# clementabary/music2dance

Measured on AMD Instinct MI355X. Metric: 120-frame seq/sec, phase3 WGAN-GP step, batch 64 per GPU, higher is better.
Workload: dtype f32

## Files before the change

music2dance_amd/build.py:

```python
import os
import shutil
import subprocess
import sys
from concurrent.futures import ThreadPoolExecutor

PKG_DIR = os.path.dirname(os.path.abspath(__file__))
CSRC = os.path.join(PKG_DIR, "csrc")
LIB_DIR = os.path.join(PKG_DIR, "lib")
LIB_PATH = os.path.join(LIB_DIR, "libm2d_hip.so")
SOURCES = ["m2d_runtime.hip", "gemm_engine.hip", "conv1d.hip", "tcn.hip", "probe_gemm.hip", "conv1d_thin.hip", "bn.hip", "gru.hip",
           "pointwise.hip", "cond.hip", "render.hip", "resample.hip", "spectral.hip"]
STAMPED = ["gemm_engine.hip", "tcn.hip"]
STAMP_LIB_PATH = os.path.join(LIB_DIR, "libm2d_hip_stamp.so")
FLAGS = ["--offload-arch=gfx950", "-O3", "-std=c++17", "-fPIC", "-ffp-contract=off", "-Wall",
         "-Wno-unused-function"] + os.environ.get("M2D_EXTRA_FLAGS", "").split()


def _hipcc():
    exe = shutil.which("hipcc") or "/opt/rocm/bin/hipcc"
    if not os.path.exists(exe):
        raise RuntimeError("hipcc not found: cannot build libm2d_hip.so")
    return exe


def _stale(target, deps):
    if not os.path.exists(target):
        return True
    t = os.path.getmtime(target)
    return any(os.path.getmtime(d) > t for d in deps)


def build(force=False, verbose=True, stamp=True):
    os.makedirs(LIB_DIR, exist_ok=True)
    obj_dir = os.path.join(LIB_DIR, "obj")
    os.makedirs(obj_dir, exist_ok=True)
    hipcc = _hipcc()
    headers = [os.path.join(CSRC, f) for f in os.listdir(CSRC) if f.endswith(".h")]
    jobs = []
    objs = []
    for src in SOURCES:
        s = os.path.join(CSRC, src)
        o = os.path.join(obj_dir, src.replace(".hip", ".o"))
        objs.append(o)
        if force or _stale(o, [s] + headers):
            jobs.append([hipcc] + FLAGS + ["-c", s, "-o", o])

    def run(cmd):
        if verbose:
            print("[m2d build]", " ".join(cmd), flush=True)
        r = subprocess.run(cmd, capture_output=True, text=True)
        if r.returncode != 0:
            raise RuntimeError("hipcc failed:\n%s\n%s" % (" ".join(cmd), r.stderr))
        return r

    sobjs = []
    sjobs = []
    if stamp:
        for src in SOURCES:
            if src in STAMPED:
                s = os.path.join(CSRC, src)
                o = os.path.join(obj_dir, src.replace(".hip", ".stamp.o"))
                sobjs.append(o)
                if force or _stale(o, [s] + headers):
                    sjobs.append([hipcc] + FLAGS + ["-DM2D_STAMP", "-c", s, "-o", o])
            else:
                sobjs.append(os.path.join(obj_dir, src.replace(".hip", ".o")))
    with ThreadPoolExecutor(max_workers=4) as ex:
        list(ex.map(run, jobs + sjobs))
    if force or jobs or _stale(LIB_PATH, objs):
        run([hipcc, "--offload-arch=gfx950", "-shared", "-fPIC", "-o", LIB_PATH] + objs)
    if stamp and (force or jobs or sjobs or _stale(STAMP_LIB_PATH, sobjs)):
        run([hipcc, "--offload-arch=gfx950", "-shared", "-fPIC", "-o", STAMP_LIB_PATH] + sobjs)
    return LIB_PATH


if __name__ == "__main__":
    build(force="--force" in sys.argv, stamp="--no-stamp" not in sys.argv)
    print(LIB_PATH)
```

music2dance_amd/csrc/conv1d.hip:

```cpp
#include "gemm_engine.h"
#include "tcn.h"

static inline int conv_out_len(int L, int ks, int stride, int pad) {
  const int span = L + 2 * pad - ks;
  return span < 0 ? 0 : span / stride + 1;
}

static inline bool fits_i32(long long v) { return v >= 0 && v < 2147483647LL; }

struct M2dWinView {
  int T, S, hop;
};
bool m2d_thin_applicable(int Cin, int Cout, int ks, int stride);
bool m2d_thin_long_applicable(int Cin, int Cout, int ks, int stride, int pad, int L);
size_t m2d_thin_long_stats_ws(int B, int Lout);
int m2d_thin_long_fwd(const float* x, const float* w, const float* bias, float* y, int B, int L, int ks, int stride, int pad,
                      int Lout, int act, float slope, const M2dWinView* wv, double* stats, void* ws, size_t ws_bytes,
                      hipStream_t stream);
size_t m2d_thin_bwd_weight_ws(int B, int Cout, int ks, int Lout);
size_t m2d_thin_fwd_stats_ws(int B, int Lout);
int m2d_thin_fwd(const float* x, const float* w, const float* bias, float* y, int B, int L, int Cout, int ks,
                 int stride, int pad, int Lout, int act, float slope, const float* out_mask, float out_mask_slope,
                 const M2dWinView* wv, double* stats, void* ws, size_t ws_bytes, hipStream_t stream);
int m2d_thin_bwd_data(const float* dy, const float* w, float* dx, int B, int L, int Cout, int ks, int stride,
                      int pad, int Lout, const float* dy_mask, float dy_mask_slope, hipStream_t stream);
int m2d_thin_bwd_weight(const float* x, const float* dy, float* dw, float* dbias, int B, int L, int Cout, int ks,
                        int stride, int pad, int Lout, const float* dy_mask, float dy_mask_slope, void* ws,
                        size_t ws_bytes, const M2dWinView* wv, hipStream_t stream);

static inline bool conv_uses_packed(int Cin) { return Cin >= M2D_BK; }
static inline float fwd_tile_penalty(int stride) { return stride > 1 ? 1.25f : 1.f; }

static void fill_fwd(M2dGemmParams& p, const float* x, const float* w, const float* wp, float* y, int B, int Cin,
                     int L, int Cout, int ks, int stride, int pad, int Lout, const M2dWinView* wv = nullptr) {
  memset(&p, 0, sizeof(p));
  p.M = Cout;
  p.N = B * Lout;
  p.K = Cin * ks;
  p.phases = 1;
  const bool packed = conv_uses_packed(Cin);
  M2dOperand& b = p.B;
  b.base = x;
  b.nbytes = m2d_extent_bytes((long long)B * Cin * L);
  b.nrows = p.N;
  b.rdiv = Lout;
  b.rdiv_inv = 1.f / (float)Lout;
  b.r_hi_stride = Cin * L;
  b.r_lo_stride = stride;
  b.r_off = -pad;
  b.r_pos_mul = stride;
  b.r_pos_off = -pad;
  b.lim = L;
  if (wv && wv->T > 0) {
    b.nbytes = m2d_extent_bytes((long long)(B / wv->T) * wv->S);
    b.r_hi_stride = wv->hop;
    b.rdiv2 = wv->T;
    b.rdiv2_inv = 1.f / (float)wv->T;
    b.r_hi2_stride = wv->S;
  }
  if (packed) {
    p.nhi = ks;
    p.kdiv = Cin;
    p.lo_outer = 1;
    p.small_tile_penalty = fwd_tile_penalty(stride);
    m2d_operand_plain(p.A, wp, Cout, 1, ks * Cout, (long long)Cout * Cin * ks);
    p.A.k_hi_stride = Cout;
    b.k_hi_stride = 1;
    b.k_lo_stride = L;
    b.k_pos_hi = 1;
    b.k_pos_lo = 0;
    b.k_safe_lo = 0;
    b.k_safe_hi = 0x7fffffff;
  } else {
    p.nhi = Cin;
    p.kdiv = ks;
    m2d_operand_plain(p.A, w, Cout, Cin * ks, 1, (long long)Cout * Cin * ks);
    p.A.k_hi_stride = ks;
    b.k_hi_stride = L;
    b.k_lo_stride = 1;
    b.k_pos_hi = 0;
    b.k_pos_lo = 1;
    b.k_safe_lo = pad;
    b.k_safe_hi = L - (Lout - 1) * stride + pad;
  }
  m2d_outmap_plain(p.O, y, Lout, 1);
  p.O.cdiv = Lout;
  p.O.cdiv_inv = 1.f / (float)Lout;
  p.O.c_hi_stride = Cout * Lout;
  p.O.c_lo_stride = 1;
}

__global__ void __launch_bounds__(256) m2d_pack_weights_kernel(const float* __restrict__ w, float* __restrict__ wf,
                                                                 float* __restrict__ wb, int Cout, int Cin, int ks) {
  const size_t total = (size_t)Cout * Cin * ks;
  for (size_t idx = (size_t)blockIdx.x * 256 + threadIdx.x; idx < total; idx += (size_t)gridDim.x * 256) {
    const int ci = (int)(idx % Cin);
    const size_t t = idx / Cin;
    const int kk = (int)(t % ks);
    const int co = (int)(t / ks);
    const float v = w[((size_t)co * Cin + ci) * ks + kk];
    if (wf) wf[idx] = v;
    if (wb) wb[((size_t)ci * ks + kk) * Cout + co] = v;
  }
}

__global__ void __launch_bounds__(256) m2d_pack_weights_subpixel_kernel(const float* __restrict__ w, float* __restrict__ out,
                                                                          int Cout, int Cin, int ks, int s, int nt, int phase_major) {
  const size_t total = (size_t)nt * Cout * Cin * s;
  for (size_t idx = (size_t)blockIdx.x * 256 + threadIdx.x; idx < total; idx += (size_t)gridDim.x * 256) {
    const int m = (int)(idx % (size_t)(Cin * s));
    const size_t k = idx / (size_t)(Cin * s);
    const int ci = phase_major ? (m / (32 * s)) * 32 + m % 32 : m / s, r = phase_major ? (m % (32 * s)) / 32 : m - ci * s;
    const int co = (int)(k % Cout), t = (int)(k / Cout);
    const int tap = r + s * t;
    out[idx] = tap < ks ? w[((size_t)co * Cin + ci) * ks + tap] : 0.f;
  }
}

static inline bool subpixel_tall(int Cin, int Cout, int ks, int stride);
static inline bool bwd_subpixel(int Cin, int Cout, int ks, int stride, bool masked_dy = false) {
  static const bool on = [] { const char* e = getenv("M2D_SUBPIXEL"); return !(e && e[0] == '0'); }();
  static const int max_rows = [] { const char* e = getenv("M2D_SUBPIXEL_MAXROWS"); return e ? atoi(e) : 128; }();
  static const int tall_max_cin = [] { const char* e = getenv("M2D_SUBPIXEL_TALL_MAXCIN"); return e ? atoi(e) : 64; }();
  if (on && !masked_dy && Cin > 32 && Cin <= tall_max_cin && subpixel_tall(Cin, Cout, ks, stride)) return true;
  return on && stride > 1 && Cin * stride <= max_rows && Cin * stride >= 64 && Cout >= 16 && ks > stride;
}
static inline bool subpixel_tall(int Cin, int Cout, int ks, int stride) {
  static const bool on = [] { const char* e = getenv("M2D_SUBPIXEL_TALL"); return !(e && e[0] == '0'); }();
  const int nt = (ks + stride - 1) / stride;
  return on && m2d_dl_enabled() && Cin % 32 == 0 && stride == 4 && ks - stride * (nt - 1) == 1 && nt >= 2;
}
static inline size_t subpixel_bytes(int Cout, int Cin, int ks, int stride) {
  return ((((size_t)((ks + stride - 1) / stride) * Cout * Cin * stride) * sizeof(float)) + 255) & ~(size_t)255;
}

static int pack_weights(const float* w, float* wf, float* wb, int Cout, int Cin, int ks, hipStream_t stream) {
  const size_t total = (size_t)Cout * Cin * ks;
  unsigned blocks = (unsigned)((total + 255) / 256);
  if (blocks > 4096) blocks = 4096;
  hipLaunchKernelGGL(m2d_pack_weights_kernel, dim3(blocks), dim3(256), 0, stream, w, wf, wb, Cout, Cin, ks);
  M2D_CHECK_LAUNCH("m2d_pack_weights_kernel");
  return M2D_OK;
}

static inline size_t pack_bytes(int Cout, int Cin, int ks) {
  return (((size_t)Cout * Cin * ks * sizeof(float)) + 255) & ~(size_t)255;
}

extern "C" {

int m2d_conv1d_pack_weights(const float* w, float* w_fwd, float* w_bwd, int Cout, int Cin, int ks, void* stream) {
  if (Cout <= 0 || Cin <= 0 || ks <= 0 || !w) M2D_FAIL(M2D_ERR_ARG, "m2d_conv1d_pack_weights: bad arguments");
  if (!fits_i32((long long)Cout * Cin * ks)) M2D_FAIL(M2D_ERR_RANGE, "m2d_conv1d_pack_weights: too large");
  if (!w_fwd && !w_bwd) return M2D_OK;
// ... 392 lines not shown
  if (stride == 1 && Lout == L && (mask_wrap % 4u) == 0) {
    const int nt = m2d_tcn_conv_tile(B, Cout, L, Cin, ks, stride, pad);
    if (nt > 0) {
      M2dTcnConv t;
      memset(&t, 0, sizeof(t));
      t.x = dy;
      t.x_mask = dy_mask;
      t.x_mask_slope = dy_mask_slope;
      t.wimg = w_packed;
      t.out = dx;
      t.out_mask = out_mask;
      t.out_mask_slope = out_mask_slope;
      t.out_mask_wrap = mask_wrap;
      t.residual = residual;
      t.mask_last = 1;
      t.tap_rev = 1;
      t.B = B;
      t.Cin = Cout;
      t.L = L;
      return m2d_tcn_conv_launch(t, ks, nt, (hipStream_t)stream, "m2d_conv1d_bwd_data");
    }
  }
  p.bwd_data = 1;
  p.plan_kind = stride > 1 ? M2D_PLAN_BWD_DATA : M2D_PLAN_GENERAL;
  p.phases = stride;
  p.ph_ks = ks;
  p.ph_cout = Cout;
  p.ph_pad = pad;
  p.ph_L = L;
  p.ph_batch = B;
  p.M = Cin;
  p.kdiv = Cout;
  p.lo_outer = 1;
  p.nhi = (ks + stride - 1) / stride;
  int nq_max = 0;
  for (int r = 0; r < stride; ++r) {
    const int qmin = r >= pad ? 0 : (pad - r + stride - 1) / stride;
    const int top = L - 1 + pad - r;
    const int nq = top >= 0 ? (top / stride - qmin + 1) : 0;
    if (nq > nq_max) nq_max = nq;
  }
  p.N = B * nq_max;
  p.K = Cout * p.nhi;
  m2d_operand_plain(p.A, w_packed, Cin, 1, ks * Cin, (long long)Cout * Cin * ks);
  p.A.k_hi_stride = stride * Cin;
  p.ph_a_step = Cin;
  M2dOperand& b = p.B;
  b.base = dy;
  b.nbytes = m2d_extent_bytes((long long)B * Cout * Lout);
  b.mask = dy_mask;
  b.mask_slope = dy_mask_slope;
  b.nrows = p.N;
  b.rdiv = nq_max;
  b.rdiv_inv = 1.f / (float)nq_max;
  b.r_hi_stride = Cout * Lout;
  b.r_lo_stride = 1;
  b.r_pos_mul = 1;
  b.k_hi_stride = -1;
  b.k_lo_stride = Lout;
  b.k_pos_hi = -1;
  b.k_pos_lo = 0;
  b.k_safe_lo = 0;
  b.k_safe_hi = 0x7fffffff;
  b.lim = Lout;
  m2d_outmap_plain(p.O, dx, L, 1);
  p.O.c_hi_stride = Cin * L;
  p.O.c_lo_stride = stride;
  p.O.c_pos_mul = stride;
  p.O.c_lim = L;
  p.O.mask = out_mask;
  p.O.mask_wrap = mask_wrap;
  p.O.mask_slope = out_mask_slope;
  p.O.residual = residual;
  p.O.mask_last = 1;
  if (stride == 1) {
    p.bwd_data = 0;
    p.phases = 1;
    p.N = B * L;
    p.nhi = ks;
    p.K = Cout * ks;
    b.nrows = p.N;
    b.rdiv = L;
    b.rdiv_inv = 1.f / (float)L;
    b.r_off = pad;
    b.r_pos_off = pad;
    p.O.cdiv = L;
    p.O.cdiv_inv = b.rdiv_inv;
    p.O.c_off = 0;
    p.O.c_pos_off = 0;
    p.O.c_lim = 0;
    return m2d_gemm_launch(p, false, false, true, ws, ws_bytes,
                           (hipStream_t)stream, "m2d_conv1d_bwd_data");
  }
  return m2d_gemm_launch(p, false, false, false, ws, ws_bytes,
                         (hipStream_t)stream, "m2d_conv1d_bwd_data");
}

int m2d_conv1d_bwd_data(const float* dy, const float* w, const float* w_packed, float* dx, int B, int Cin, int L,
                        int Cout, int ks, int stride, int pad, const float* dy_mask, float dy_mask_slope,
                        const float* out_mask, float out_mask_slope, void* ws, size_t ws_bytes, void* stream) {
  return conv1d_bwd_data_impl(dy, w, w_packed, dx, B, Cin, L, Cout, ks, stride, pad, dy_mask, dy_mask_slope, out_mask,
                              out_mask_slope, ws, ws_bytes, stream, nullptr);
}

int m2d_conv1d_bwd_data_res(const float* dy, const float* w, const float* w_packed, float* dx, int B, int Cin, int L,
                            int Cout, int ks, int stride, int pad, const float* dy_mask, float dy_mask_slope,
                            const float* residual, const float* out_mask, float out_mask_slope, void* ws,
                            size_t ws_bytes, void* stream) {
  return conv1d_bwd_data_impl(dy, w, w_packed, dx, B, Cin, L, Cout, ks, stride, pad, dy_mask, dy_mask_slope, out_mask,
                              out_mask_slope, ws, ws_bytes, stream, residual);
}

int m2d_conv1d_bwd_data_shared_mask(const float* dy, const float* w, const float* w_packed, float* dx, int B, int Cin,
                                    int L, int Cout, int ks, int stride, int pad, const float* out_mask,
                                    float out_mask_slope, int mask_batch, void* ws, size_t ws_bytes, void* stream) {
  if (m2d_thin_applicable(Cin, Cout, ks, stride))
    M2D_FAIL(M2D_ERR_ARG, "m2d_conv1d_bwd_data_shared_mask: not for the thin (Cin = 1) layer");
  return conv1d_bwd_data_impl(dy, w, w_packed, dx, B, Cin, L, Cout, ks, stride, pad, nullptr, 0.f, out_mask,
                              out_mask_slope, ws, ws_bytes, stream, nullptr, mask_batch);
}

static int conv1d_bwd_weight_impl(const float* x, const float* dy, float* dw, float* dbias, int B, int Cin, int L,
                                  int Cout, int ks, int stride, int pad, const float* dy_mask, float dy_mask_slope,
                                  void* ws, size_t ws_bytes, void* stream, const M2dWinView* wv,
                                  int bias_from_sample = 0) {
  const int Lout = conv_out_len(L, ks, stride, pad);
  if (bias_from_sample < 0 || bias_from_sample > B) M2D_FAIL(M2D_ERR_ARG, "m2d_conv1d_bwd_weight: bad bias_from_sample");
  if (bias_from_sample > 0 && dbias && (Lout < M2D_BK || m2d_thin_applicable(Cin, Cout, ks, stride)))
    M2D_FAIL(M2D_ERR_ARG, "m2d_conv1d_bwd_weight: bias_from_sample needs >= %d output positions and Cin > 1", M2D_BK);
  if (B <= 0 || Cin <= 0 || Cout <= 0 || Lout <= 0)
    M2D_FAIL(M2D_ERR_ARG, "m2d_conv1d_bwd_weight: bad shape");
  if (!fits_i32((long long)B * Cin * L) || !fits_i32((long long)B * Cout * Lout))
    M2D_FAIL(M2D_ERR_RANGE, "m2d_conv1d_bwd_weight: tensor exceeds 2^31 elements");
  if (m2d_thin_applicable(Cin, Cout, ks, stride))
    return m2d_thin_bwd_weight(x, dy, dw, dbias, B, L, Cout, ks, stride, pad, Lout, dy_mask, dy_mask_slope, ws,
                               ws_bytes, wv, (hipStream_t)stream);
  if (wv && (Cin != 1 || Lout < M2D_BK))
    M2D_FAIL(M2D_ERR_ARG, "m2d_conv1d_bwd_weight_windows: single-channel convs with >= %d output positions only", M2D_BK);
  if (!wv && Lout == L && m2d_tcn_wgrad_applicable(B, Cin, L, Cout, ks, stride, pad)) {
    M2dTcnWgrad t;
    memset(&t, 0, sizeof(t));
    t.x = x;
    t.dy = dy;
    t.dy_mask = dy_mask;
    t.dy_mask_slope = dy_mask_slope;
    t.dw = dw;
    t.dbias = dbias;
    t.bias_from = bias_from_sample;
    t.B = B;
    t.Cin = Cin;
    t.L = L;
    return m2d_tcn_wgrad_launch(t, ks, ws, ws_bytes, (hipStream_t)stream, "m2d_conv1d_bwd_weight");
  }
  M2dGemmParams p;
  memset(&p, 0, sizeof(p));
  p.M = Cout;
  p.N = Cin * ks;
  p.K = B * Lout;
  p.phases = 1;
  M2dOperand& b = p.B;
  b.base = x;
  b.nbytes = m2d_extent_bytes((long long)B * Cin * L);
  b.nrows = p.N;
  b.rdiv = ks;
  b.rdiv_inv = 1.f / (float)ks;
  b.r_hi_stride = L;
  b.r_lo_stride = 1;
  b.r_off = -pad;
  b.r_pos_mul = 1;
  b.r_pos_off = -pad;
  b.lim = L;
  bool a_kfast = true;
  if (Lout >= M2D_BK) {
    p.nhi = B;
    p.kdiv = Lout;
    m2d_operand_plain(p.A, dy, Cout, Lout, 1, (long long)B * Cout * Lout);
    p.A.k_hi_stride = Cout * Lout;
    b.k_hi_stride = Cin * L;
    b.k_lo_stride = stride;
    b.k_pos_hi = 0;
    b.k_pos_lo = stride;
    if (wv && wv->T > 0) {
      b.nbytes = m2d_extent_bytes((long long)(B / wv->T) * wv->S);
      b.k_hi_stride = wv->hop;
      b.kdiv2 = wv->T;
      b.k_hi2_stride = wv->S;
    }
    b.k_safe_lo = (pad + stride - 1) / stride;
    b.k_safe_hi = (L - ks + pad) >= 0 ? (L - ks + pad) / stride + 1 : 0;
    p.plan_kind = M2D_PLAN_BWD_WEIGHT;
  } else {
    p.nhi = Lout;
    p.kdiv = B;
    a_kfast = false;
    m2d_operand_plain(p.A, dy, Cout, Lout, Cout * Lout, (long long)B * Cout * Lout);
    p.A.k_hi_stride = 1;
    b.k_hi_stride = stride;
    b.k_lo_stride = Cin * L;
    b.k_pos_hi = stride;
    b.k_pos_lo = 0;
    b.k_safe_lo = 0;
    b.k_safe_hi = 0x7fffffff;
  }
  p.A.mask = dy_mask;
  p.A.mask_slope = dy_mask_slope;
  m2d_outmap_plain(p.O, dw, Cin * ks, 1);
  if (dbias) {
    p.N = Cin * ks + 1;
    b.ones_row_p1 = Cin * ks + 1;
    b.ones_from_hi = bias_from_sample;
    p.O.col_out = dbias;
    p.O.redirect_col_p1 = Cin * ks + 1;
  }
  return m2d_gemm_launch(p, a_kfast, false, true, ws, ws_bytes, (hipStream_t)stream,
                         "m2d_conv1d_bwd_weight");
}

int m2d_conv1d_bwd_weight(const float* x, const float* dy, float* dw, float* dbias, int B, int Cin, int L,
                          int Cout, int ks, int stride, int pad, const float* dy_mask, float dy_mask_slope,
                          void* ws, size_t ws_bytes, void* stream) {
  return conv1d_bwd_weight_impl(x, dy, dw, dbias, B, Cin, L, Cout, ks, stride, pad, dy_mask, dy_mask_slope, ws,
                                ws_bytes, stream, nullptr);
}

int m2d_conv1d_bwd_weight_from(const float* x, const float* dy, float* dw, float* dbias, int B, int Cin, int L,
                               int Cout, int ks, int stride, int pad, const float* dy_mask, float dy_mask_slope,
                               int bias_from_sample, void* ws, size_t ws_bytes, void* stream) {
  return conv1d_bwd_weight_impl(x, dy, dw, dbias, B, Cin, L, Cout, ks, stride, pad, dy_mask, dy_mask_slope, ws,
                                ws_bytes, stream, nullptr, bias_from_sample);
}

int m2d_conv1d_bwd_weight_windows(const float* track, int B, int S, int T, int hop, int window, const float* dy,
                                  float* dw, float* dbias, int Cout, int ks, int stride, int pad,
                                  const float* dy_mask, float dy_mask_slope, void* ws, size_t ws_bytes, void* stream) {
  if (B <= 0 || T <= 0 || hop <= 0 || window <= 0 || (long long)(T - 1) * hop + window > S)
    M2D_FAIL(M2D_ERR_ARG, "m2d_conv1d_bwd_weight_windows: windows do not fit the track");
  if (!fits_i32((long long)B * S) || !fits_i32((long long)B * T * window))
    M2D_FAIL(M2D_ERR_RANGE, "m2d_conv1d_bwd_weight_windows: tensor exceeds 2^31 elements");
  const M2dWinView wv = {T, S, hop};
  return conv1d_bwd_weight_impl(track, dy, dw, dbias, B * T, 1, window, Cout, ks, stride, pad, dy_mask, dy_mask_slope,
                                ws, ws_bytes, stream, &wv);
}

size_t m2d_conv1d_workspace_bytes(int which, int B, int Cin, int L, int Cout, int ks, int stride, int pad) {
  const int Lout = conv_out_len(L, ks, stride, pad);
  if (Lout <= 0) return 0;
  if (m2d_thin_applicable(Cin, Cout, ks, stride))
    return which == 2 ? m2d_thin_bwd_weight_ws(B, Cout, ks, Lout) : (which == 0 ? m2d_thin_fwd_stats_ws(B, Lout) : 0);
  if (which == 0 && m2d_thin_long_applicable(Cin, Cout, ks, stride, pad, L)) {
    const size_t a = m2d_gemm_plan(Cout, B * Lout, m2d_chunks(Cin, ks), 1, true).ws_bytes + m2d_rowstats_bytes(Cout, B * Lout);
    const size_t t = m2d_thin_long_stats_ws(B, Lout);
    return a > t ? a : t;
  }
  if (which == 0) {
    if (Lout == 1 && pad == 0 && L == ks) {
      const size_t a = m2d_gemm_plan(Cout, B, m2d_chunks(1, Cin * ks), 1, true).ws_bytes, st = m2d_rowstats_bytes(Cout, B);
      return a + st;
    }
    const bool packed = conv_uses_packed(Cin);
    const int nch = packed ? m2d_chunks(ks, Cin) : m2d_chunks(Cin, ks);
    const size_t a = m2d_gemm_plan(Cout, B * Lout, nch, 1, true, packed ? fwd_tile_penalty(stride) : 1.f).ws_bytes;
    const size_t st = m2d_rowstats_bytes(Cout, B * Lout);
    return a + st + (packed ? pack_bytes(Cout, Cin, ks) : 0);
  }
  if (which == 1) {
    if (Lout == 1 && pad == 0 && L == ks) return m2d_gemm_plan(B, Cin * ks, m2d_chunks(1, Cout), 1, true).ws_bytes;
    if (stride == 1) return m2d_gemm_plan(Cin, B * L, m2d_chunks(ks, Cout), 1, true).ws_bytes + pack_bytes(Cout, Cin, ks);
    if (bwd_subpixel(Cin, Cout, ks, stride)) return subpixel_bytes(Cout, Cin, ks, stride) + pack_bytes(Cout, Cin, ks);
    return pack_bytes(Cout, Cin, ks);
  }
  const int nch = Lout >= M2D_BK ? m2d_chunks(B, Lout) : m2d_chunks(Lout, B);
  const int kind = Lout >= M2D_BK ? M2D_PLAN_BWD_WEIGHT : M2D_PLAN_GENERAL;
  const size_t a = m2d_gemm_plan(Cout, Cin * ks, nch, 1, true, 1.0, kind).ws_bytes;
  const size_t c = m2d_gemm_plan(Cout, Cin * ks + 1, nch, 1, true, 1.0, kind).ws_bytes;
  const size_t t = (Lout == L && m2d_tcn_wgrad_applicable(B, Cin, L, Cout, ks, stride, pad)) ? m2d_tcn_wgrad_ws_bytes(B, Cin, L, ks) : 0;
  return (a > c ? a : c) > t ? (a > c ? a : c) : t;
}

static int gemm_impl(int mode, const float* a, int lda, const float* b, int ldb, const float* bias, float* c, int ldc,
                     int M, int N, int K, int act, float slope, const float* a_mask, float a_mask_slope,
                     const float* out_mask, float out_mask_slope, void* ws, size_t ws_bytes, void* stream) {
  if (M < 0 || N < 0 || K < 0 || mode < 0 || mode > 2) M2D_FAIL(M2D_ERR_ARG, "m2d_gemm: bad arguments");
  const int a_cols = mode == 2 ? M : K, b_cols = mode == 0 ? K : N;
  if (lda == 0) lda = a_cols;
  if (ldb == 0) ldb = b_cols;
  if (ldc == 0) ldc = N;
  if (lda < a_cols || ldb < b_cols || ldc < N) M2D_FAIL(M2D_ERR_ARG, "m2d_gemm: leading dimension smaller than the row");
  if (!fits_i32((long long)M * K) || !fits_i32((long long)N * K) || !fits_i32((long long)M * N))
    M2D_FAIL(M2D_ERR_RANGE, "m2d_gemm: matrix exceeds 2^31 elements");
  M2dGemmParams p;
  memset(&p, 0, sizeof(p));
  p.M = M;
  p.N = N;
  p.K = K;
  p.nhi = K > 0 ? 1 : 0;
  p.kdiv = K > 0 ? K : 1;
  p.phases = 1;
  bool akf = true, bkf = true;
  const long long a_rows = mode == 2 ? K : M, b_rows = mode == 0 ? N : K;
  const long long ea = K > 0 ? (a_rows - 1) * lda + a_cols : 1, eb = K > 0 ? (b_rows - 1) * ldb + b_cols : 1;
  if (!fits_i32((long long)(M - 1) * ldc + N)) M2D_FAIL(M2D_ERR_RANGE, "m2d_gemm: output exceeds 2^31 elements");
  if (mode == 0) {
    m2d_operand_plain(p.A, a, M, lda, 1, ea);
    m2d_operand_plain(p.B, b, N, ldb, 1, eb);
    akf = true;
    bkf = true;
  } else if (mode == 1) {
    m2d_operand_plain(p.A, a, M, lda, 1, ea);
    m2d_operand_plain(p.B, b, N, 1, ldb, eb);
    akf = true;
    bkf = false;
  } else {
    m2d_operand_plain(p.A, a, M, 1, lda, ea);
    m2d_operand_plain(p.B, b, N, 1, ldb, eb);
    akf = false;
    bkf = false;
  }
  p.A.mask = a_mask;
  p.A.mask_slope = a_mask_slope;
  m2d_outmap_plain(p.O, c, ldc, 1);
  p.O.bias = bias;
  p.O.bias_mode = bias ? 2 : 0;
  p.O.act = act;
  p.O.slope = slope;
  p.O.mask = out_mask;
  p.O.mask_slope = out_mask_slope;
  return m2d_gemm_launch(p, akf, bkf, true, ws, ws_bytes, (hipStream_t)stream, "m2d_gemm");
}

int m2d_gemm(int mode, const float* a, const float* b, const float* bias, float* c, int M, int N, int K,
             int act, float slope, const float* a_mask, float a_mask_slope, const float* out_mask,
             float out_mask_slope, void* ws, size_t ws_bytes, void* stream) {
  return gemm_impl(mode, a, 0, b, 0, bias, c, 0, M, N, K, act, slope, a_mask, a_mask_slope, out_mask, out_mask_slope,
                   ws, ws_bytes, stream);
}

int m2d_gemm_ld(int mode, const float* a, int lda, const float* b, int ldb, const float* bias, float* c, int ldc,
                int M, int N, int K, int act, float slope, const float* a_mask, float a_mask_slope,
                const float* out_mask, float out_mask_slope, void* ws, size_t ws_bytes, void* stream) {
  return gemm_impl(mode, a, lda, b, ldb, bias, c, ldc, M, N, K, act, slope, a_mask, a_mask_slope, out_mask,
                   out_mask_slope, ws, ws_bytes, stream);
}

size_t m2d_gemm_workspace_bytes(int mode, int M, int N, int K) {
  (void)mode;
  return m2d_gemm_plan(M, N, m2d_chunks(K > 0 ? 1 : 0, K > 0 ? K : 1), 1, true).ws_bytes;
}

}
```

Baseline: 5702.

## Add specialized MFMA weight-gradient kernel for k25 stride-4 conv1d

Adds a dedicated weight-gradient kernel for conv1d layers with kernel size 25, stride 4 and padding 11 (the WaveGAN-style discriminator shape). It uses fp32 32x32x2 MFMA with double-buffered LDS staging of dy and x chunks, buffer loads with out-of-bounds handling, and a per-run partial slab. A separate reduce kernel then sums the partials into dw and dbias. It replaces the generic GEMM-engine path for these shapes, adds workspace sizing for the new slab, and can be disabled with an env var. The cost is more code and a two-kernel split-K reduction.

After: 5731 (median of 6 runs). Within noise of the previous version (+0.5%).

```diff
diff --git a/music2dance_amd/build.py b/music2dance_amd/build.py
--- a/music2dance_amd/build.py
+++ b/music2dance_amd/build.py
@@ -8,7 +8,8 @@
 CSRC = os.path.join(PKG_DIR, "csrc")
 LIB_DIR = os.path.join(PKG_DIR, "lib")
 LIB_PATH = os.path.join(LIB_DIR, "libm2d_hip.so")
-SOURCES = ["m2d_runtime.hip", "gemm_engine.hip", "conv1d.hip", "tcn.hip", "probe_gemm.hip", "conv1d_thin.hip", "bn.hip", "gru.hip",
+SOURCES = ["m2d_runtime.hip", "gemm_engine.hip", "conv1d.hip", "tcn.hip", "conv1d_wgrad_k4.hip", "probe_gemm.hip", "conv1d_thin.hip",
+           "bn.hip", "gru.hip",
            "pointwise.hip", "cond.hip", "render.hip", "resample.hip", "spectral.hip"]
 STAMPED = ["gemm_engine.hip", "tcn.hip"]
 STAMP_LIB_PATH = os.path.join(LIB_DIR, "libm2d_hip_stamp.so")
diff --git a/music2dance_amd/csrc/conv1d.hip b/music2dance_amd/csrc/conv1d.hip
--- a/music2dance_amd/csrc/conv1d.hip
+++ b/music2dance_amd/csrc/conv1d.hip
@@ -1,5 +1,6 @@
 #include "gemm_engine.h"
 #include "tcn.h"
+#include "conv1d_wgrad_k4.h"
 
 static inline int conv_out_len(int L, int ks, int stride, int pad) {
   const int span = L + 2 * pad - ks;
@@ -698,6 +699,22 @@
     t.L = L;
     return m2d_tcn_wgrad_launch(t, ks, ws, ws_bytes, (hipStream_t)stream, "m2d_conv1d_bwd_weight");
   }
+  if (!wv && m2d_wgrad_k4_applicable(B, Cin, L, Cout, ks, stride, pad, dbias != nullptr)) {
+    M2dWgradK4 t;
+    memset(&t, 0, sizeof(t));
+    t.x = x;
+    t.dy = dy;
+    t.dy_mask = dy_mask;
+    t.dy_mask_slope = dy_mask_slope;
+    t.dw = dw;
+    t.dbias = dbias;
+    t.bias_from = bias_from_sample;
+    t.B = B;
+    t.Cin = Cin;
+    t.L = L;
+    t.Cout = Cout;
+    return m2d_wgrad_k4_launch(t, ws, ws_bytes, (hipStream_t)stream, "m2d_conv1d_bwd_weight");
+  }
   M2dGemmParams p;
   memset(&p, 0, sizeof(p));
   p.M = Cout;
@@ -820,7 +837,14 @@
   const size_t a = m2d_gemm_plan(Cout, Cin * ks, nch, 1, true, 1.0, kind).ws_bytes;
   const size_t c = m2d_gemm_plan(Cout, Cin * ks + 1, nch, 1, true, 1.0, kind).ws_bytes;
   const size_t t = (Lout == L && m2d_tcn_wgrad_applicable(B, Cin, L, Cout, ks, stride, pad)) ? m2d_tcn_wgrad_ws_bytes(B, Cin, L, ks) : 0;
-  return (a > c ? a : c) > t ? (a > c ? a : c) : t;
+  size_t k4 = 0;
+  for (int wb = 0; wb < 2; ++wb)
+    if (m2d_wgrad_k4_applicable(B, Cin, L, Cout, ks, stride, pad, wb)) {
+      const size_t b = m2d_wgrad_k4_ws_bytes(B, Cin, L, Cout, wb);
+      k4 = b > k4 ? b : k4;
+    }
+  const size_t e = (a > c ? a : c) > t ? (a > c ? a : c) : t;
+  return e > k4 ? e : k4;
 }
 
 static int gemm_impl(int mode, const float* a, int lda, const float* b, int ldb, const float* bias, float* c, int ldc,
diff --git a/music2dance_amd/csrc/conv1d_wgrad_k4.h b/music2dance_amd/csrc/conv1d_wgrad_k4.h
--- /dev/null
+++ b/music2dance_amd/csrc/conv1d_wgrad_k4.h
@@ -0,0 +1,16 @@
+#pragma once
+#include "m2d_common.h"
+
+struct M2dWgradK4 {
+  const float* x;
+  const float* dy;
+  const float* dy_mask;
+  float dy_mask_slope;
+  float* dw;
+  float* dbias;
+  int bias_from;
+  int B, Cin, L, Cout;
+};
+int m2d_wgrad_k4_applicable(int B, int Cin, int L, int Cout, int ks, int stride, int pad, int with_bias);
+size_t m2d_wgrad_k4_ws_bytes(int B, int Cin, int L, int Cout, int with_bias);
+int m2d_wgrad_k4_launch(const M2dWgradK4& p, void* ws, size_t ws_bytes, hipStream_t stream, const char* what);
diff --git a/music2dance_amd/csrc/conv1d_wgrad_k4.hip b/music2dance_amd/csrc/conv1d_wgrad_k4.hip
--- /dev/null
+++ b/music2dance_amd/csrc/conv1d_wgrad_k4.hip
@@ -0,0 +1,369 @@
+#include "conv1d_wgrad_k4.h"
+#include "gemm_engine.h"
+
+#include <stdlib.h>
+#include <type_traits>
+
+typedef float wk4_f32x16 __attribute__((ext_vector_type(16)));
+typedef float wk4_f32x4 __attribute__((ext_vector_type(4)));
+
+#define WK4_OOB 0x80000000u
+
+static __device__ __forceinline__ __amdgpu_buffer_rsrc_t wk4_rsrc(const void* p, unsigned nbytes) {
+  return __builtin_amdgcn_make_buffer_rsrc((void*)p, (short)0, (int)nbytes, 0x00020000);
+}
+static __device__ __forceinline__ wk4_f32x4 wk4_bload4(__amdgpu_buffer_rsrc_t r, unsigned voff) {
+  return __builtin_bit_cast(wk4_f32x4, __builtin_amdgcn_raw_buffer_load_b128(r, (int)voff, 0, 0));
+}
+static __device__ __forceinline__ unsigned wk4_lds_addr(const float* p) {
+  return (unsigned)(uintptr_t)(__attribute__((address_space(3))) const float*)p;
+}
+template <int OFF>
+static __device__ __forceinline__ float wk4_ds_read(unsigned addr) {
+  float v;
+  asm volatile("ds_read_b32 %0, %1 offset:%2" : "=v"(v) : "v"(addr), "n"(OFF));
+  return v;
+}
+template <int I, int N, class F>
+static __device__ __forceinline__ void wk4_static_for(F&& f) {
+  if constexpr (I < N) {
+    f(std::integral_constant<int, I>{});
+    wk4_static_for<I + 1, N>(f);
+  }
+}
+
+struct Wk4Tile {
+  static constexpr int KS = 25;
+  static constexpr int ROWS = 64;
+  static constexpr int TILE4 = 2 * KS * 4 * 64;
+  static constexpr size_t part_floats() { return (size_t)TILE4 * 4 + ROWS; }
+};
+template <int KCR_>
+struct Wk4Cfg : Wk4Tile {
+  static constexpr int KCR = KCR_;
+  static constexpr int KC = (KCR + 1) & ~1;
+  static constexpr int LDD = KC | 1;
+  static constexpr int XP = KC + 6;
+  static constexpr int XW = 4 * XP;
+  static constexpr int LDXW = XW | 1;
+  static constexpr int XIMG = ROWS * LDD;
+  static constexpr int STAGE_DATA = XIMG + 32 * LDXW;
+  static constexpr int STAGE = STAGE_DATA + 16;
+  static constexpr int AHEAD = 2;
+  static constexpr int NSTEP = KC / 2;
+  static constexpr size_t lds_bytes() { return (size_t)2 * STAGE * sizeof(float) + 64; }
+};
+
+struct Wk4Plan {
+  int ncg;
+  int nrg;
+  int nck;
+  int cpw;
+  int nr;
+};
+static int wk4_plan(int B, int Cin, int L, int Cout, int with_bias, Wk4Plan* out) {
+  const int Lout = L / 4;
+  if (Lout % 240 != 0) return 0;
+  const int nch = m2d_chunks(B, Lout);
+  const int splits = m2d_gemm_plan(Cout, Cin * Wk4Tile::KS + (with_bias ? 1 : 0), nch, 1, true, 1.0, M2D_PLAN_BWD_WEIGHT).splits;
+  if (splits > 1 && splits <= 16) return 0;
+  const int cps = (nch + splits - 1) / splits;
+  if ((cps * M2D_BK) % 60 != 0) return 0;
+  Wk4Plan q;
+  q.ncg = Cin / 32;
+  q.nrg = (Cout + Wk4Tile::ROWS - 1) / Wk4Tile::ROWS;
+  q.nck = B * (Lout / 60);
+  q.cpw = cps * M2D_BK / 60;
+  q.nr = (q.nck + q.cpw - 1) / q.cpw;
+  if ((long long)q.ncg * q.nrg * q.nr > 256) return 0;
+  if (out) *out = q;
+  return 1;
+}
+
+template <int KCR, int NT, bool DMASK>
+static __device__ __forceinline__ void wk4_run(const M2dWgradK4& p, float* __restrict__ part, float* smem, int cpw, int nck,
+                                               int r, int rb, int cg, int rg, int run) {
+  using Cfg = Wk4Cfg<KCR>;
+  constexpr int KC = Cfg::KC, LDD = Cfg::LDD, XP = Cfg::XP, LDXW = Cfg::LDXW, STAGE = Cfg::STAGE, XIMG = Cfg::XIMG;
+  constexpr int AHEAD = Cfg::AHEAD, NSTEP = Cfg::NSTEP;
+  const int tid = threadIdx.x;
+  const int lane = tid & 63;
+  const int l31 = lane & 31, lh = lane >> 5;
+  const int L = p.L, Cin = p.Cin, Cout = p.Cout;
+  const int Lout = L >> 2;
+  const int cpl = Lout / KCR;
+  const int ck0 = run * cpw;
+  const int ck1 = ck0 + cpw < nck ? ck0 + cpw : nck;
+
+  const unsigned dy_bytes = (unsigned)((size_t)p.B * Cout * Lout * sizeof(float));
+  const __amdgpu_buffer_rsrc_t rdy = wk4_rsrc(p.dy, dy_bytes);
+  const __amdgpu_buffer_rsrc_t rmk = wk4_rsrc(DMASK ? p.dy_mask : p.dy, DMASK ? dy_bytes : 0u);
+  const __amdgpu_buffer_rsrc_t rx = wk4_rsrc(p.x, (unsigned)((size_t)p.B * Cin * L * sizeof(float)));
+
+  constexpr bool FLAT = KCR % 4 != 0;
+  constexpr int NPDY = Cfg::ROWS * KCR / 4;
+  constexpr int NDY = (NPDY + 511) / 512;
+  constexpr int NX = (32 * XP + 511) / 512;
+  unsigned dy_off[NDY];
+  int dy_lds[NDY][FLAT ? 4 : 1];
+  unsigned x_off[NX];
+  int x_pos[NX], x_lds[NX];
+#pragma unroll
+  for (int i = 0; i < NDY; ++i) {
+    const int e = tid + 512 * i;
+    const bool in = e < NPDY;
+    if constexpr (!FLAT) {
+      const int row = e / (KCR / 4), c4 = e - row * (KCR / 4);
+      const int co = rg * Cfg::ROWS + row;
+      dy_off[i] = (in && co < Cout) ? (unsigned)((co * Lout + 4 * c4) * 4) : WK4_OOB;
+      dy_lds[i][0] = in ? row * LDD + 4 * c4 : Cfg::STAGE_DATA;
+    } else {
+      const int rows = Cout - rg * Cfg::ROWS < Cfg::ROWS ? Cout - rg * Cfg::ROWS : Cfg::ROWS;
+      dy_off[i] = (in && 4 * e < rows * KCR) ? (unsigned)((rg * Cfg::ROWS * KCR + 4 * e) * 4) : WK4_OOB;
+#pragma unroll
+      for (int j = 0; j < 4; ++j) {
+        const int row = (4 * e + j) / KCR, col = 4 * e + j - row * KCR;
+        dy_lds[i][j] = in ? row * LDD + col : Cfg::STAGE_DATA + j;
+      }
+    }
+  }
+#pragma unroll
+  for (int i = 0; i < NX; ++i) {
+    const int e = tid + 512 * i;
+    const int ci = e / XP, c4 = e - ci * XP;
+    const bool in = e < 32 * XP;
+    x_off[i] = in ? (unsigned)(((cg * 32 + ci) * L) * 4) : WK4_OOB;
+    x_pos[i] = 4 * c4 - 12;
+    x_lds[i] = in ? XIMG + ci * LDXW + 4 * c4 : Cfg::STAGE_DATA + 4;
+  }
+  wk4_f32x4 rdv[NDY], rmv[DMASK ? NDY : 1], rxv[NX];
+  auto load_chunk = [&](int ck) {
+    const int n = ck / cpl, lc0 = (ck - n * cpl) * KCR;
+    const unsigned dbase = (unsigned)((n * Cout * Lout + lc0) * 4);
+#pragma unroll
+    for (int i = 0; i < NDY; ++i) {
+      const unsigned off = dy_off[i] != WK4_OOB ? dy_off[i] + dbase : WK4_OOB;
+      rdv[i] = wk4_bload4(rdy, off);
+      if constexpr (DMASK) rmv[i] = wk4_bload4(rmk, off);
+    }
+    const unsigned xbase = (unsigned)((n * Cin * L) * 4);
+#pragma unroll
+    for (int i = 0; i < NX; ++i) {
+      const int pos = 4 * lc0 + x_pos[i];
+      const bool ok = x_off[i] != WK4_OOB && (unsigned)pos < (unsigned)L;
+      rxv[i] = wk4_bload4(rx, ok ? x_off[i] + xbase + (unsigned)(pos * 4) : WK4_OOB);
+    }
+  };
+  auto store_chunk = [&](float* st) {
+    const float ms = p.dy_mask_slope;
+#pragma unroll
+    for (int i = 0; i < NDY; ++i) {
+      wk4_f32x4 v = rdv[i];
+      if constexpr (DMASK) {
+#pragma unroll
+        for (int j = 0; j < 4; ++j) v[j] *= (rmv[i][j] > 0.f ? 1.f : ms);
+      }
+#pragma unroll
+      for (int j = 0; j < 4; ++j) st[FLAT ? dy_lds[i][j] : dy_lds[i][0] + j] = v[j];
+    }
+#pragma unroll
+    for (int i = 0; i < NX; ++i)
+#pragma unroll
+      for (int j = 0; j < 4; ++j) st[x_lds[i] + j] = rxv[i][j];
+  };
+
+  wk4_f32x16 acc[NT];
+#pragma unroll
+  for (int j = 0; j < NT; ++j)
+#pragma unroll
+    for (int q = 0; q < 16; ++q) acc[j][q] = 0.f;
+  const bool do_bias = cg == 0 && p.dbias != nullptr && (tid >> 6) == 2;
+  float bsum = 0.f;
+
+  const unsigned a_base = wk4_lds_addr(smem) + (unsigned)(((rb * 32 + l31) * LDD + lh) * 4);
+  const unsigned b_base = wk4_lds_addr(smem) + (unsigned)((XIMG + l31 * LDXW + 4 * lh + r + 1) * 4);
+
+  if constexpr (KC != KCR) {
+    if (tid < 2 * Cfg::ROWS) smem[(tid >> 6) * STAGE + (tid & 63) * LDD + KCR] = 0.f;
+  }
+  if (ck0 < ck1) {
+    load_chunk(ck0);
+    store_chunk(smem);
+  }
+  asm volatile("s_waitcnt lgkmcnt(0)" ::: "memory");
+  __builtin_amdgcn_s_barrier();
+
+  constexpr int NW = 2 * NSTEP + NT - 1;
+  for (int ck = ck0; ck < ck1; ++ck) {
+    const int cur = (ck - ck0) & 1;
+    load_chunk(ck + 1 < ck1 ? ck + 1 : ck);
+    __builtin_amdgcn_sched_barrier(0);
+    const unsigned aa = a_base + (unsigned)(cur * STAGE * 4), bb = b_base + (unsigned)(cur * STAGE * 4);
+    float fa[NSTEP], fw[NW];
+    auto issue_frag = [&](auto S_) {
+      constexpr int S = decltype(S_)::value;
+      fa[S] = wk4_ds_read<2 * S * 4>(aa);
+      if constexpr (S == 0) {
+        wk4_static_for<0, NT>([&](auto j_) { fw[decltype(j_)::value] = wk4_ds_read<decltype(j_)::value * 16>(bb); });
+      } else {
+        fw[2 * S + NT - 2] = wk4_ds_read<(2 * S + NT - 2) * 16>(bb);
+        fw[2 * S + NT - 1] = wk4_ds_read<(2 * S + NT - 1) * 16>(bb);
+      }
+    };
+    auto staging = [&]() {
+      asm volatile("s_waitcnt lgkmcnt(0)" ::: "memory");
+      __builtin_amdgcn_sched_barrier(0);
+      if (do_bias && ck / cpl >= p.bias_from) {
+        const float* drow = smem + cur * STAGE + (tid & 63) * LDD;
+#pragma unroll
+        for (int k = 0; k < KCR; ++k) bsum += drow[k];
+      }
+      store_chunk(smem + (cur ^ 1) * STAGE);
+      asm volatile("s_waitcnt lgkmcnt(0)" ::: "memory");
+      __builtin_amdgcn_sched_barrier(0);
+    };
+    constexpr int STAGE_AT0 = NSTEP / 4, STAGE_AT1 = (3 * NSTEP) / 4;
+    wk4_static_for<0, AHEAD>([&](auto s_) { issue_frag(s_); });
+    wk4_static_for<0, NSTEP>([&](auto s_) {
+      constexpr int S = decltype(s_)::value;
+      if constexpr (S + AHEAD < NSTEP) issue_frag(std::integral_constant<int, S + AHEAD>{});
+      constexpr int LEFT = (S + AHEAD < NSTEP ? AHEAD : NSTEP - 1 - S) * 3;
+      asm volatile("s_waitcnt lgkmcnt(%3)" : "+v"(fa[S]), "+v"(fw[2 * S + NT - 2]), "+v"(fw[2 * S + NT - 1]) : "n"(LEFT));
+#pragma unroll
+      for (int j = 0; j < NT; ++j) acc[j] = __builtin_amdgcn_mfma_f32_32x32x2f32(fa[S], fw[2 * S + j], acc[j], 0, 0, 0);
+      __builtin_amdgcn_sched_barrier(0);
+      if constexpr (S == STAGE_AT0) {
+        if (rb == 0) staging();
+      }
+      if constexpr (S == STAGE_AT1) {
+        if (rb == 1) staging();
+      }
+    });
+    asm volatile("s_waitcnt lgkmcnt(0)" ::: "memory");
+    __builtin_amdgcn_s_barrier();
+  }
+
+  wk4_f32x4* dst = reinterpret_cast<wk4_f32x4*>(part);
+#pragma unroll
+  for (int j = 0; j < NT; ++j)
+#pragma unroll
+    for (int q = 0; q < 4; ++q) {
+      const wk4_f32x4 v = {acc[j][4 * q], acc[j][4 * q + 1], acc[j][4 * q + 2], acc[j][4 * q + 3]};
+      dst[((rb * Cfg::KS + r + 4 * j) * 4 + q) * 64 + lane] = v;
+    }
+  if ((tid >> 6) == 2) part[(size_t)Cfg::TILE4 * 4 + (tid & 63)] = bsum;
+}
+
+template <int KCR, bool DMASK>
+__global__ void __launch_bounds__(512, 1) m2d_wgrad_k4_kernel(const M2dWgradK4 p, float* __restrict__ slab, int cpw, int nck, int ncg) {
+  extern __shared__ __attribute__((aligned(16))) float smem[];
+  const int wave = __builtin_amdgcn_readfirstlane(threadIdx.x >> 6);
+  const int rb = wave >> 2, r = (wave & 3) ^ rb;
+  const int g = blockIdx.x, run = blockIdx.y;
+  const int rg = g / ncg, cg = g - rg * ncg;
+  float* part = slab + (size_t)(run * gridDim.x + g) * Wk4Tile::part_floats();
+  if (r == 0) wk4_run<KCR, 7, DMASK>(p, part, smem, cpw, nck, r, rb, cg, rg, run);
+  else wk4_run<KCR, 6, DMASK>(p, part, smem, cpw, nck, r, rb, cg, rg, run);
+}
+
+__global__ void __launch_bounds__(256) m2d_wgrad_k4_reduce_kernel(const float* __restrict__ slab, float* __restrict__ dw,
+                                                                    float* __restrict__ dbias, int nr, int Cin, int Cout, int ncg) {
+  using Cfg = Wk4Tile;
+  __shared__ wk4_f32x4 sh[8][32];
+  const int g = blockIdx.x, ng = gridDim.x;
+  const int rg = g / ncg, cg = g - rg * ncg;
+  const size_t pf = Cfg::part_floats();
+  const int tid = threadIdx.x;
+  if (blockIdx.y == Cfg::TILE4 / 32) {
+    if (!dbias || cg != 0) return;
+    const int m = tid & 63, jj = tid >> 6;
+    const float* src = slab + (size_t)g * pf + (size_t)Cfg::TILE4 * 4 + m;
+    float* shb = reinterpret_cast<float*>(sh);
+#pragma unroll
+    for (int h = 0; h < 2; ++h) {
+      float c = 0.f;
+      for (int z = jj + 4 * h; z < nr; z += 8) c += src[(size_t)z * ng * pf];
+      shb[(jj + 4 * h) * 64 + m] = c;
+    }
+    __syncthreads();
+    const int co = rg * Cfg::ROWS + m;
+    if (jj == 0 && co < Cout)
+      dbias[co] = ((shb[m] + shb[64 + m]) + (shb[128 + m] + shb[192 + m])) + ((shb[256 + m] + shb[320 + m]) + (shb[384 + m] + shb[448 + m]));
+    return;
+  }
+  const int ul = tid & 31, j = tid >> 5;
+  const int u = blockIdx.y * 32 + ul;
+  wk4_f32x4 c = {0.f, 0.f, 0.f, 0.f};
+  const wk4_f32x4* src = reinterpret_cast<const wk4_f32x4*>(slab + (size_t)g * pf) + u;
+  const size_t stride4 = (size_t)ng * pf / 4;
+#pragma unroll 4
+  for (int z = j; z < nr; z += 8) c += src[(size_t)z * stride4];
+  sh[j][ul] = c;
+  __syncthreads();
+  if (j > 0) return;
+  const wk4_f32x4 s = ((sh[0][ul] + sh[1][ul]) + (sh[2][ul] + sh[3][ul])) + ((sh[4][ul] + sh[5][ul]) + (sh[6][ul] + sh[7][ul]));
+  const int lane = u & 63, tq = u >> 6, q = tq & 3, tt = tq >> 2;
+  const int rb = tt / Cfg::KS, t = tt - rb * Cfg::KS;
+  const int ci = cg * 32 + (lane & 31);
+#pragma unroll
+  for (int i = 0; i < 4; ++i) {
+    const int co = rg * Cfg::ROWS + rb * 32 + i + 8 * q + 4 * (lane >> 5);
+    if (co < Cout) dw[((size_t)co * Cin + ci) * Cfg::KS + t] = s[i];
+  }
+}
+
+int m2d_wgrad_k4_applicable(int B, int Cin, int L, int Cout, int ks, int stride, int pad, int with_bias) {
+  const char* e = getenv("M2D_WGRAD_K4");
+  if (e && e[0] == '0') return 0;
+  if (ks != Wk4Tile::KS || stride != 4 || pad != 11 || B <= 0 || Cin <= 0 || Cout <= 0 || L <= 0) return 0;
+  if (L % 4 != 0 || Cin % 32 != 0 || Cout % 32 != 0) return 0;
+  if ((long long)B * Cin * L >= (1LL << 29) || (long long)B * Cout * (L / 4) >= (1LL << 29)) return 0;
+  return wk4_plan(B, Cin, L, Cout, with_bias, nullptr);
+}
+
+extern "C" int m2d_debug_wgrad_k4_runs(int B, int Cin, int L, int Cout, int with_bias) {
+  Wk4Plan q;
+  if (!m2d_wgrad_k4_applicable(B, Cin, L, Cout, Wk4Tile::KS, 4, 11, with_bias) || !wk4_plan(B, Cin, L, Cout, with_bias, &q)) return 0;
+  return q.nr;
+}
+
+size_t m2d_wgrad_k4_ws_bytes(int B, int Cin, int L, int Cout, int with_bias) {
+  Wk4Plan q;
+  if (!wk4_plan(B, Cin, L, Cout, with_bias, &q)) return 0;
+  return (size_t)q.nr * q.ncg * q.nrg * Wk4Tile::part_floats() * sizeof(float) + 256;
+}
+
+int m2d_wgrad_k4_launch(const M2dWgradK4& p, void* ws, size_t ws_bytes, hipStream_t stream, const char* what) {
+  using Cfg = Wk4Tile;
+  const int with_bias = p.dbias ? 1 : 0;
+  Wk4Plan q;
+  if (!m2d_wgrad_k4_applicable(p.B, p.Cin, p.L, p.Cout, Cfg::KS, 4, 11, with_bias) || !wk4_plan(p.B, p.Cin, p.L, p.Cout, with_bias, &q))
+    M2D_FAIL(M2D_ERR_ARG, "%s: not a shape of the k25 / stride-4 kernel", what);
+  const size_t need = m2d_wgrad_k4_ws_bytes(p.B, p.Cin, p.L, p.Cout, with_bias);
+  if (!ws || ws_bytes < need) M2D_FAIL(M2D_ERR_WORKSPACE, "%s: workspace too small (%zu < %zu)", what, ws_bytes, need);
+  if (((uintptr_t)p.x | (uintptr_t)p.dy | (uintptr_t)p.dy_mask) & 15) M2D_FAIL(M2D_ERR_ARG, "%s: the k25 / stride-4 kernel needs 16-byte aligned tensors", what);
+  float* slab = reinterpret_cast<float*>(((uintptr_t)ws + 255) & ~(uintptr_t)255);
+  const int Lout = p.L / 4;
+  const int ncols = p.Cin * Cfg::KS + with_bias;
+  const double flops = 2.0 * p.Cout * (double)p.B * Lout * ncols;
+  M2dProfScope prof(M2D_FAM_GEMM, stream, flops, 0.0, what, p.Cout, ncols, p.B * Lout);
+  const size_t lds = Wk4Cfg<60>::lds_bytes();
+  const int groups = q.ncg * q.nrg;
+  auto go = [&](auto kern) -> int {
+    static bool attr_set = false;
+    if (!attr_set) {
+      if (hipFuncSetAttribute(reinterpret_cast<const void*>(kern), hipFuncAttributeMaxDynamicSharedMemorySize, 160 * 1024) != hipSuccess)
+        M2D_FAIL(M2D_ERR_HIP, "%s: cannot raise the dynamic LDS limit", what);
+      attr_set = true;
+    }
+    hipLaunchKernelGGL(kern, dim3(groups, q.nr), dim3(512), lds, stream, p, slab, q.cpw, q.nck, q.ncg);
+    return M2D_OK;
+  };
+  const int rc = p.dy_mask ? go(m2d_wgrad_k4_kernel<60, true>) : go(m2d_wgrad_k4_kernel<60, false>);
+  if (rc) return rc;
+  M2D_CHECK_LAUNCH(what);
+  hipLaunchKernelGGL(m2d_wgrad_k4_reduce_kernel, dim3(groups, Cfg::TILE4 / 32 + 1), dim3(256), 0, stream, slab, p.dw, p.dbias, q.nr,
+                     p.Cin, p.Cout, q.ncg);
+  M2D_CHECK_LAUNCH(what);
+  return M2D_OK;
+}
```
